# elicassion/active-gym

Hardware: NVIDIA B200
Metric: foveal_obs_per_sec (higher is better)
Workload: dtype u8

## Files before the change

active_gym_b200/csrc/agym_device.cuh:

```cuda
#pragma once
#include "agym_kernels.cuh"
#ifndef AGYM_EXPERIMENT
#define AGYM_EXPERIMENT 0
#endif

#include <cuda.h>
#include <cuda_bf16.h>
#include <cuda_fp16.h>

#include <algorithm>
#include <utility>
#include <cstdlib>
#include <cstring>

#include "../../include/agym_b200.h"

namespace agym {

namespace {


constexpr int kThreads = 256;

__device__ __forceinline__ uint4 ld_stream128(const void *p) {
// ... 126 lines not shown

__device__ __forceinline__ uint4 luma16(const uint32_t (&w)[12], uint32_t w01, uint32_t w2) {
    uint32_t acc[16];
#pragma unroll
    for (int i = 0; i < 16; ++i) {
        const int j = 3 * i, wi = j >> 2, b = j & 3;
        const uint32_t hi = wi + 1 < 12 ? w[wi + 1] : 0u;
        const uint32_t q = __byte_perm(w[wi], hi, (uint32_t)(b | (b + 1) << 4 | (b + 2) << 8 | 0x4000));
        acc[i] = __dp2a_hi(w2, q, __dp2a_lo(w01, q, 32768u));
    }
    uint32_t o[4];
#pragma unroll
    for (int m = 0; m < 4; ++m)
        o[m] = __byte_perm(__byte_perm(acc[4 * m], acc[4 * m + 1], 0x0062), __byte_perm(acc[4 * m + 2], acc[4 * m + 3], 0x0062), 0x5410);
    return make_uint4(o[0], o[1], o[2], o[3]);
}

__device__ __forceinline__ size_t align16(size_t v) { return (v + 15) & ~size_t(15); }

constexpr float kBias = 49152.5f;

__device__ void squeeze_to_cache(const DevPlan &p, const uint8_t *s_frame, float *s_t1, float *dst_global, int tid, int nt) {
    resample_w<uint8_t>(s_frame, p.S_w, s_t1, p.p_w, p.S_h, p.sq_w, tid, nt);
    __syncthreads();
    resample_h<float>(s_t1, p.p_w, dst_global, p.p_w, p.p_w, p.sq_h, tid, nt);
}

__device__ __forceinline__ uint32_t smem_u32(const void *p) { return (uint32_t)__cvta_generic_to_shared(p); }
__device__ __forceinline__ void mbar_init(uint64_t *bar, uint32_t count) {
    asm volatile("mbarrier.init.shared::cta.b64 [%0], %1;" ::"r"(smem_u32(bar)), "r"(count));
}
__device__ __forceinline__ void mbar_fence_init() { asm volatile("fence.mbarrier_init.release.cluster;" ::: "memory"); }
__device__ __forceinline__ void mbar_expect_tx(uint64_t *bar, uint32_t bytes) {
    asm volatile("mbarrier.arrive.expect_tx.shared::cta.b64 _, [%0], %1;" ::"r"(smem_u32(bar)), "r"(bytes) : "memory");
}
constexpr uint32_t kBackoffNs = 2000;
template <bool BACKOFF = false>
__device__ __forceinline__ void mbar_wait(uint64_t *bar, uint32_t parity) {
    uint32_t done = 0;
    while (!done) {
        if (BACKOFF) {
            asm volatile(
                "{\n\t.reg .pred p;\n\t"
                "mbarrier.try_wait.parity.shared::cta.b64 p, [%1], %2, %3;\n\t"
                "selp.u32 %0, 1, 0, p;\n\t}"
                : "=r"(done)
                : "r"(smem_u32(bar)), "r"(parity), "r"(kBackoffNs)
                : "memory");
        } else {
            asm volatile(
                "{\n\t.reg .pred p;\n\t"
                "mbarrier.try_wait.parity.shared::cta.b64 p, [%1], %2;\n\t"
                "selp.u32 %0, 1, 0, p;\n\t}"
                : "=r"(done)
                : "r"(smem_u32(bar)), "r"(parity)
                : "memory");
        }
    }
}
__device__ __forceinline__ void bulk_g2s(void *smem_dst, const void *gmem_src, uint32_t bytes, uint64_t *bar) {
    asm volatile("cp.async.bulk.shared::cluster.global.mbarrier::complete_tx::bytes [%0], [%1], %2, [%3];" ::"r"(
                     smem_u32(smem_dst)),
                 "l"(gmem_src), "r"(bytes), "r"(smem_u32(bar))
                 : "memory");
}

__device__ __forceinline__ void tensor_g2s_4d(void *smem_dst, const CUtensorMap *map, uint64_t *bar, int c0, int c1, int c2, int c3) {
    asm volatile("cp.async.bulk.tensor.4d.shared::cluster.global.mbarrier::complete_tx::bytes [%0], [%1, {%3, %4, %5, %6}], [%2];" ::"r"(
                     smem_u32(smem_dst)),
                 "l"(reinterpret_cast<uint64_t>(map)), "r"(smem_u32(bar)), "r"(c0), "r"(c1), "r"(c2), "r"(c3)
                 : "memory");
}

__device__ __forceinline__ void bulk_s2g(void *gmem_dst, const void *smem_src, uint32_t bytes) {
    asm volatile("cp.async.bulk.global.shared::cta.bulk_group [%0], [%1], %2;" ::"l"(gmem_dst), "r"(smem_u32(smem_src)),
                 "r"(bytes)
                 : "memory");
}
__device__ __forceinline__ void bulk_commit() { asm volatile("cp.async.bulk.commit_group;" ::: "memory"); }
template <int N>
__device__ __forceinline__ void bulk_wait_read() { asm volatile("cp.async.bulk.wait_group.read %0;" ::"n"(N) : "memory"); }
__device__ __forceinline__ void fence_async_smem() { asm volatile("fence.proxy.async.shared::cta;" ::: "memory"); }

__device__ __forceinline__ void mbar_arrive(uint64_t *bar) {
    asm volatile("mbarrier.arrive.shared::cta.b64 _, [%0];" ::"r"(smem_u32(bar)) : "memory");
}
__device__ __forceinline__ void consumer_sync() { asm volatile("bar.sync 1, %0;" ::"n"(kThreads) : "memory"); }

__device__ __forceinline__ void pdl_launch_dependents() { asm volatile("griddepcontrol.launch_dependents;" ::: "memory"); }
__device__ __forceinline__ void pdl_wait() { asm volatile("griddepcontrol.wait;" ::: "memory"); }

__device__ __forceinline__ void cp_async16(void *smem_dst, const void *gmem_src) {
    asm volatile("cp.async.cg.shared.global [%0], [%1], 16;" ::"r"((uint32_t)__cvta_generic_to_shared(smem_dst)), "l"(gmem_src));
}
__device__ __forceinline__ void cp_async16_s(uint32_t smem_addr, const void *gmem_src) {
    asm volatile("cp.async.cg.shared.global [%0], [%1], 16;" ::"r"(smem_addr), "l"(gmem_src));
}
__device__ __forceinline__ void cp_async4(void *smem_dst, const void *gmem_src) {
    asm volatile("cp.async.ca.shared.global [%0], [%1], 4;" ::"r"((uint32_t)__cvta_generic_to_shared(smem_dst)), "l"(gmem_src));
}
__device__ __forceinline__ void cp_async4_s(uint32_t smem_addr, const void *gmem_src) {
    asm volatile("cp.async.ca.shared.global [%0], [%1], 4;" ::"r"(smem_addr), "l"(gmem_src));
}
template <int SOFF, int GOFF>
__device__ __forceinline__ void cp_async4_imm(uint32_t smem_addr, const void *gmem_src) {
    asm volatile("cp.async.ca.shared.global [%0 + %2], [%1 + %3], 4;" ::"r"(smem_addr), "l"(gmem_src), "n"(SOFF), "n"(GOFF));
}
__device__ __forceinline__ void cp_async_commit() { asm volatile("cp.async.commit_group;" ::: "memory"); }
template <int N>
__device__ __forceinline__ void cp_async_wait() { asm volatile("cp.async.wait_group %0;" ::"n"(N) : "memory"); }

__device__ __forceinline__ float norm_u8(uint32_t u) {
    const float x = (float)u, r = 1.0f / 255.0f;
    const float q0 = x * r;
    return fmaf(fmaf(-q0, 255.0f, x), r, q0);
}
__device__ __forceinline__ void norm_store4(int dt, uint32_t word, void *dst, size_t index) {
    const float f0 = norm_u8(word & 0xffu), f1 = norm_u8((word >> 8) & 0xffu), f2 = norm_u8((word >> 16) & 0xffu), f3 = norm_u8(word >> 24);
    if (dt == AGYM_DTYPE_F32) {
        reinterpret_cast<float4 *>(dst)[index] = make_float4(f0, f1, f2, f3);
    } else if (dt == AGYM_DTYPE_F16) {
        const __half2 a = __floats2half2_rn(f0, f1), b = __floats2half2_rn(f2, f3);
        reinterpret_cast<uint2 *>(dst)[index] = make_uint2(*reinterpret_cast<const uint32_t *>(&a), *reinterpret_cast<const uint32_t *>(&b));
    } else {
        const __nv_bfloat162 a = __floats2bfloat162_rn(f0, f1), b = __floats2bfloat162_rn(f2, f3);
        reinterpret_cast<uint2 *>(dst)[index] = make_uint2(*reinterpret_cast<const uint32_t *>(&a), *reinterpret_cast<const uint32_t *>(&b));
    }
}
__device__ __forceinline__ void norm_store16(int dt, const uint4 v, void *dst, size_t index) {
    const uint32_t w[4] = {v.x, v.y, v.z, v.w};
    if (dt == AGYM_DTYPE_F32) {
        float4 *o = reinterpret_cast<float4 *>(dst) + 4 * index;
#pragma unroll
        for (int j = 0; j < 4; ++j)
            o[j] = make_float4(norm_u8(w[j] & 0xffu), norm_u8((w[j] >> 8) & 0xffu), norm_u8((w[j] >> 16) & 0xffu), norm_u8(w[j] >> 24));
    } else {
        uint32_t h[8];
#pragma unroll
        for (int j = 0; j < 4; ++j) {
            const float f0 = norm_u8(w[j] & 0xffu), f1 = norm_u8((w[j] >> 8) & 0xffu), f2 = norm_u8((w[j] >> 16) & 0xffu), f3 = norm_u8(w[j] >> 24);
            if (dt == AGYM_DTYPE_F16) {
                const __half2 a = __floats2half2_rn(f0, f1), b = __floats2half2_rn(f2, f3);
                h[2 * j] = *reinterpret_cast<const uint32_t *>(&a); h[2 * j + 1] = *reinterpret_cast<const uint32_t *>(&b);
            } else {
                const __nv_bfloat162 a = __floats2bfloat162_rn(f0, f1), b = __floats2bfloat162_rn(f2, f3);
                h[2 * j] = *reinterpret_cast<const uint32_t *>(&a); h[2 * j + 1] = *reinterpret_cast<const uint32_t *>(&b);
            }
        }
        uint4 *o = reinterpret_cast<uint4 *>(dst) + 2 * index;
        o[0] = make_uint4(h[0], h[1], h[2], h[3]);
        o[1] = make_uint4(h[4], h[5], h[6], h[7]);
    }
}

__device__ __forceinline__ uint64_t pack2(float lo, float hi) {
    uint64_t r;
    asm("mov.b64 %0, {%1, %2};" : "=l"(r) : "f"(lo), "f"(hi));
    return r;
}
__device__ __forceinline__ void unpack2(uint64_t v, uint32_t &lo, uint32_t &hi) {
    asm("mov.b64 {%0, %1}, %2;" : "=r"(lo), "=r"(hi) : "l"(v));
}
__device__ __forceinline__ uint64_t ffma2(uint64_t a, uint64_t b, uint64_t c) {
    uint64_t d;
    asm("fma.rn.f32x2 %0, %1, %2, %3;" : "=l"(d) : "l"(a), "l"(b), "l"(c));
    return d;
}
__device__ __forceinline__ uint64_t fsub2(uint64_t a, uint64_t b) {
    uint64_t d;
    asm("sub.rn.f32x2 %0, %1, %2;" : "=l"(d) : "l"(a), "l"(b));
// ... 43 lines not shown
```

active_gym_b200/csrc/agym_observe.cu:

```cuda
#include "agym_device.cuh"

namespace agym {

namespace {

template <int VARIANT>
__global__ void __launch_bounds__(kThreads) k_observe_fixed(const __grid_constant__ DevPlan p,
                                                            const uint8_t *__restrict__ ring,
                                                            const int32_t *__restrict__ head,
                                                            const double *__restrict__ action,
                                                            const uint8_t *__restrict__ ctrl, int32_t *__restrict__ loc,
                                                            uint8_t *__restrict__ out) {
    extern __shared__ __align__(16) uint8_t smem[];
    __shared__ int s_loc[2];
    const int n = blockIdx.x, tid = threadIdx.x;
    if (tid == 0) {
        int r, c;
        update_loc_fixed(p, n, action, ctrl, loc, r, c);
        s_loc[0] = r; s_loc[1] = c;
    }
    __syncthreads();
    const int r0 = s_loc[0], c0 = s_loc[1];
    const int h = head[n];
    const uint8_t *env_ring = ring + (size_t)n * p.K * p.plane;
// ... 473 lines not shown
            const float *s = sq + a_part * p.p_w;
            float *t = s_T + a_part * S_w + 2 * cp;
            const int sstep = parts * p.p_w, tstep = parts * S_w;
#pragma unroll 4
            for (int r = a_part; r < trows; r += parts, s += sstep, t += tstep) {
                const uint64_t u = pack2(s[a_i0], s[a_i1]), v = pack2(s[a_i0 + 1], s[a_i1 + 1]);
                *reinterpret_cast<uint64_t *>(t) = ffma2(a_w0, u, ffma2(a_w1, v, bias2));
            }
        }
        __syncthreads();

        if (active) {
            const uint32_t *fvb = reinterpret_cast<const uint32_t *>(sq + sq_words);
            const uint32_t fov_mask = word_mask(4 * q, lc, lc + p.f_w);
            const int rf = fov_mask ? lr : (1 << 29);
            const int fstride = f_h * nw_max;
            for (int k0 = 0; k0 < K; k0 += KG) {
                uint32_t *orow = out_w + ((size_t)e * K + k0) * wpp + (uint32_t)y_begin * quads + q;
                const uint32_t *fv = fvb + (k0 * f_h - rf) * nw_max + (q - (lc >> 2));
                const float *tk = s_T + (size_t)k0 * p.p_h * S_w + 4 * q;
                const int kstride = p.p_h * S_w;
                int y = y_begin, j_have = -2;
                const int2 *rp = s_row + y_begin;
                int2 rw = *rp;
                uint64_t b0[KG], b1[KG], d0[KG], d1[KG];
                while (y < y_end) {
                    const int j0 = rw.x;
#pragma unroll
                    for (int kk = 0; kk < KG; ++kk) {
                        const float *tj = tk + kk * kstride + j0 * S_w;
                        uint64_t a0, a1;
                        if (j0 == j_have + 1) { a0 = b0[kk]; a1 = b1[kk]; }
                        else { const ulonglong2 a = *reinterpret_cast<const ulonglong2 *>(tj); a0 = a.x; a1 = a.y; }
                        const ulonglong2 b = *reinterpret_cast<const ulonglong2 *>(tj + S_w);
                        b0[kk] = b.x; b1[kk] = b.y;
                        d0[kk] = fsub2(a0, b.x); d1[kk] = fsub2(a1, b.y);
                    }
                    j_have = j0;
                    do {
                        const float w0 = __int_as_float(rw.y);
                        const uint64_t w2 = pack2(w0, w0);
                        rw = *++rp;
                        uint32_t word[KG];
#pragma unroll
                        for (int kk = 0; kk < KG; ++kk) {
                            uint32_t u0, u1, u2, u3;
                            unpack2(ffma2(w2, d0[kk], b0[kk]), u0, u1);
                            unpack2(ffma2(w2, d1[kk], b1[kk]), u2, u3);
                            word[kk] = __byte_perm(__byte_perm(u0, u1, 0x0051), __byte_perm(u2, u3, 0x0051), 0x5410);
                        }
                        if ((unsigned)(y - rf) < (unsigned)f_h) {
                            const uint32_t *sh = fv + y * nw_max;
#pragma unroll
                            for (int kk = 0; kk < KG; ++kk) word[kk] = (word[kk] & ~fov_mask) | (sh[kk * fstride] & fov_mask);
                        }
#pragma unroll
                        for (int kk = 0; kk < KG; ++kk) orow[kk * wpp] = word[kk];
                        orow += quads;
                        ++y;
                    } while (rw.x == j0 && y < y_end);
                }
            }
        }
        __syncthreads();
        lr = lr1; lc = lc1; hh = hh1; hh1 = hh2;
        lr1 = s_loc[it & 1][0]; lc1 = s_loc[it & 1][1];
    }
}

struct StdGeom {
    static constexpr int S = 84, P = 20, Q = 21, SEG = 4, R = 21, SPAN = 7;
    __host__ __device__ static constexpr int src(int i) { return (40 * i - 64 + 168 * 4) / 168 - 4; }
};

template <int NW, int R0>
__device__ __forceinline__ void prefetch_rows_imm(uint32_t rows, uint32_t dst, const uint32_t *src) {
    if constexpr (R0 < StdGeom::R) {
        if (rows & (1u << R0)) cp_async4_imm<R0 * (NW ? NW : 1) * 4, R0 * StdGeom::Q * 4>(dst, src);
        prefetch_rows_imm<NW, R0 + 1>(rows, dst, src);
    }
}

template <int K, int NW, bool FS>
__global__ void __launch_bounds__(((StdGeom::Q * StdGeom::SEG * K + 31) / 32) * 32, 2)
    k_observe_peripheral_std(const __grid_constant__ DevPlan p, const __grid_constant__ ExpandStd ew,
                             const uint8_t *__restrict__ ring, const int32_t *__restrict__ head,
                             const float *__restrict__ pcache, const double *__restrict__ action,
                             const uint8_t *__restrict__ ctrl, int32_t *__restrict__ loc, uint8_t *__restrict__ out) {
    using Gm = StdGeom;
    constexpr int S = Gm::S, P = Gm::P, Q = Gm::Q, R = Gm::R;
    constexpr int NB = Q * Gm::SEG * K;
    constexpr int PP = P * P, PLANE_W = S * S / 4;
    constexpr int NBUF = 3, DIST = 2, LOC_RING = 128;
    extern __shared__ __align__(16) uint8_t smem[];
    __shared__ int4 s_loc[LOC_RING];
    __shared__ __align__(8) uint64_t full[NBUF];
    const int tid = threadIdx.x;
    const int N = p.N, f_h = p.f_h, f_w = p.f_w, G = gridDim.x;
    const int nw_max = NW ? NW : (f_w + 3) / 4 + 1;
    const int rowbuf = (f_h * Q + 9) & ~3;
    const int buf_words = K * PP + (FS ? K * rowbuf : ((K * f_h * nw_max + 3) & ~3));
    float *bufs = reinterpret_cast<float *>(smem);
    uint32_t *tiles = reinterpret_cast<uint32_t *>(bufs + NBUF * buf_words);
    const uint32_t *ring_w = reinterpret_cast<const uint32_t *>(ring);

    auto loc_batch = [&](int it0) {
        const int j = it0 + (tid & 31);
        const int env = j <= N / G + 1 ? (int)blockIdx.x + j * G : N;
        int r = 0, c = 0, hh = 0;
        if (env < N) {
            update_loc_fixed<true>(p, env, action, ctrl, loc, r, c);
            hh = head[env];
        }
        s_loc[j & (LOC_RING - 1)] = make_int4(r, c, hh, 0);
    };
    pdl_launch_dependents();
    if (tid == 0) {
        for (int i = 0; i < NBUF; ++i) mbar_init(&full[i], 1);
        mbar_fence_init();
    }

    const bool active = tid < NB;
    const int q = tid % Q, t2 = tid / Q;
    constexpr int kOrd4[16] = {7, 4, 13, 3, 0, 1, 9, 6, 10, 14, 11, 12, 8, 5, 15, 2};
    constexpr int kOrd3[12] = {11, 8, 5, 2, 9, 6, 3, 0, 10, 4, 1, 7};
    const int grp = !active ? 0 : (K == 4 ? kOrd4[t2 & 15] : (K == 3 ? kOrd3[t2 % 12] : t2));
    const int g = grp % Gm::SEG, k = grp / Gm::SEG;
    int base;
    uint64_t wa01, wa23, wb01, wb23, wc01, wc23;
    {
        const int i00 = __ldg(p.exw_i0 + 4 * q);
        base = min(i00, P - 3);
        float wa[4], wb[4], wc[4];
#pragma unroll
        for (int c = 0; c < 4; ++c) {
            const int sel = __ldg(p.exw_i0 + 4 * q + c) - base;
            const float w0 = __ldg(p.exw_w0 + 4 * q + c), w1 = __ldg(p.exw_w1 + 4 * q + c);
            wa[c] = sel == 0 ? w0 : 0.f;
            wb[c] = sel == 0 ? w1 : w0;
            wc[c] = sel == 0 ? 0.f : w1;
        }
        wa01 = pack2(wa[0], wa[1]); wa23 = pack2(wa[2], wa[3]);
        wb01 = pack2(wb[0], wb[1]); wb23 = pack2(wb[2], wb[3]);
        wc01 = pack2(wc[0], wc[1]); wc23 = pack2(wc[2], wc[3]);
    }
    const uint64_t bias2 = pack2(kBias, kBias);
    const int row_first = 5 * g - 1;
    const int so_t0 = (row_first < 0 ? 0 : row_first) * P + base;
    const int so_mid = row_first * P + base;
    const int so_t6 = (row_first + 6 > P - 1 ? P - 1 : row_first + 6) * P + base;
    const uint32_t bufs_s = smem_u32(bufs);
    const uint32_t word0 = (uint32_t)(g * R) * Q + q;
    constexpr int NJ = 2;
    int ck_row[NJ], ck_k[NJ], ck_c4[NJ];
    if constexpr (FS) {
        const int cpr = (f_w + 14) / 16 + 1, total = K * f_h * cpr;
#pragma unroll
        for (int a = 0; a < NJ; ++a) {
            const int i = tid + a * (int)blockDim.x;
            const int row = i / cpr, kk = row / f_h;
            ck_k[a] = i < total ? kk : -1;
            ck_row[a] = (row - kk * f_h) * Q;
            ck_c4[a] = (i - row * cpr) * 4;
        }
    }

    auto fovea_rows = [&](int lr, int lc, uint32_t &mask) {
        mask = word_mask(4 * q, lc, lc + f_w);
        const int r_lo = lr - g * R;
        const int m_lo = max(r_lo, 0), m_hi = min(r_lo + f_h, R);
        return (mask && m_hi > m_lo) ? (((1u << m_hi) - 1u) & ~((1u << m_lo) - 1u)) : 0u;
    };
    auto fovea_pos = [&](int lr, int lc) { return (k * f_h + g * R - lr) * nw_max + (q - (lc >> 2)); };
    auto prefetch = [&](int env, int j) {
        const int b = j % NBUF;
        if (tid == 0) {
            mbar_expect_tx(&full[b], K * PP * 4);
            bulk_g2s(bufs + b * buf_words, pcache + (size_t)env * (K * PP), K * PP * 4, &full[b]);
        }
        if constexpr (FS) {
            const int4 lh = s_loc[j & (LOC_RING - 1)];
            const int top = lh.x * Q, wb = top & ~3;
            const int lw = lh.y >> 2, lastw = (lh.y + f_w - 1) >> 2;
#pragma unroll
            for (int a = 0; a < NJ; ++a) {
                if (ck_k[a] < 0) continue;
                const int rowbase = top + ck_row[a];
                const int cw = ((rowbase + lw) & ~3) + ck_c4[a];
                if (cw > rowbase + lastw) continue;
                int slot = lh.z + 1 + ck_k[a];
                slot -= slot >= K ? K : 0;
                cp_async16_s(bufs_s + (uint32_t)(b * buf_words + K * PP + ck_k[a] * rowbuf + (cw - wb)) * 4u,
                             ring_w + ((size_t)env * K + slot) * PLANE_W + cw);
            }
        } else if (active) {
            const int4 lh = s_loc[j & (LOC_RING - 1)];
            uint32_t mask;
            const uint32_t rows = fovea_rows(lh.x, lh.y, mask);
            if (rows) {
                int slot = lh.z + 1 + k;
                slot -= slot >= K ? K : 0;
                const uint32_t *src = ring_w + ((size_t)env * K + slot) * PLANE_W + word0;
                const uint32_t dst = bufs_s + (uint32_t)(b * buf_words + K * PP + fovea_pos(lh.x, lh.y)) * 4u;
                if (NW) {
                    prefetch_rows_imm<NW, 0>(rows, dst, src);
                } else {
#pragma unroll
                    for (int r = 0; r < R; ++r)
                        if (rows & (1u << r)) cp_async4_s(dst + (uint32_t)(r * nw_max) * 4u, src + r * Q);
                }
            }
        }
    };
    auto t_row = [&](const float *sq, int so, uint64_t &t01, uint64_t &t23) {
        const float s0 = sq[so], s1 = sq[so + 1], s2 = sq[so + 2];
        const uint64_t p0 = pack2(s0, s0), p1 = pack2(s1, s1), p2 = pack2(s2, s2);
        t01 = ffma2(p2, wc01, ffma2(p1, wb01, ffma2(p0, wa01, bias2)));
        t23 = ffma2(p2, wc23, ffma2(p1, wb23, ffma2(p0, wa23, bias2)));
    };

    pdl_wait();
    if (tid < 32) loc_batch(0);
    __syncthreads();
    {
        const int e0 = blockIdx.x;
#pragma unroll
        for (int j = 0; j < DIST; ++j) {
            if (e0 + j * G < N) prefetch(e0 + j * G, j);
            cp_async_commit();
        }
        if constexpr (FS) {
            cp_async_wait<DIST - 1>();
            __syncthreads();
        }
    }
    int it = 0;
    for (int e = blockIdx.x; e < N; e += G, ++it) {
        if (e + DIST * G < N) prefetch(e + DIST * G, it + DIST);
        cp_async_commit();
        if ((it & 31) == 0 && tid < 32) loc_batch(it + 32);
        const int b = it % NBUF;
        if constexpr (!FS) cp_async_wait<DIST>();
        mbar_wait(&full[b], (it / NBUF) & 1);
        uint32_t *tile = tiles + (it & 1) * (K * PLANE_W);
        if (active) {
            const int4 lh = s_loc[it & (LOC_RING - 1)];
            uint32_t fov_mask;
            const uint32_t rows = fovea_rows(lh.x, lh.y, fov_mask);
            int slot = lh.z + 1 + k;
            slot -= slot >= K ? K : 0;
            const float *sq = bufs + b * buf_words + slot * PP;
            const uint32_t *sh = reinterpret_cast<const uint32_t *>(bufs + b * buf_words + K * PP) +
                                 (FS ? k * rowbuf + (int)word0 - ((lh.x * Q) & ~3) : fovea_pos(lh.x, lh.y));
            constexpr int SHP = FS ? Q : 0;
            uint32_t *o = tile + k * PLANE_W + word0;
            uint64_t a0, a1, b0, b1, d0 = 0, d1 = 0;
            t_row(sq, so_t0, a0, a1);
            t_row(sq, so_mid + P, b0, b1);
            int t_have = 0;
#pragma unroll
            for (int r = 0; r < R; ++r) {
                const int t = Gm::src(r) + 1;
                if (t != t_have) {
                    a0 = b0; a1 = b1;
                    t_row(sq, t + 1 == Gm::SPAN - 1 ? so_t6 : so_mid + (t + 1) * P, b0, b1);
                    t_have = t;
                }
                if (r == 0 || Gm::src(r) != Gm::src(r - 1)) { d0 = fsub2(a0, b0); d1 = fsub2(a1, b1); }
                const uint64_t w2 = pack2(ew.hw[r], ew.hw[r]);
                uint32_t u0, u1, u2, u3;
                unpack2(ffma2(w2, d0, b0), u0, u1);
                unpack2(ffma2(w2, d1, b1), u2, u3);
                uint32_t word = __byte_perm(__byte_perm(u0, u1, 0x0051), __byte_perm(u2, u3, 0x0051), 0x5410);
                if (rows & (1u << r))
                    word = (word & ~fov_mask) | (sh[FS ? r * SHP : r * nw_max] & fov_mask);
                o[r * Q] = word;
            }
        }
        fence_async_smem();
        if (tid == 0) bulk_wait_read<0>();
        if constexpr (FS) cp_async_wait<DIST - 1>();
        __syncthreads();
        if (tid == 0) {
            bulk_s2g(out + (size_t)e * (K * PLANE_W * 4), tile, K * PLANE_W * 4);
            bulk_commit();
        }
        if (p.norm_out) {
            const uint4 *t4 = reinterpret_cast<const uint4 *>(tile);
            for (int i = tid; i < K * PLANE_W / 4; i += (int)blockDim.x)
                norm_store16(p.norm_dt, t4[i], p.norm_out, (size_t)e * (K * PLANE_W / 4) + i);
        }
    }
    if (tid == 0) bulk_wait_read<0>();
}


}

namespace {
cudaError_t normalize_after(cudaError_t e, const uint8_t *out, size_t bytes, void *norm_out, int norm_dt, cudaStream_t st) {
    if (e != cudaSuccess || !norm_out) return e;
    if (bytes % 16 != 0) return cudaErrorInvalidValue;
    return launch_normalize(out, bytes, norm_dt, norm_out, st);
}
}

cudaError_t launch_observe_fixed(const DevPlan &p0, const uint8_t *ring, const int32_t *head, const double *action,
                                 const uint8_t *ctrl, int32_t *loc, int variant, uint8_t *out, void *norm_out, int norm_dt,
                                 cudaStream_t st) {
    DevPlan p = p0;
    p.norm_out = norm_out; p.norm_dt = norm_dt;
    const size_t out_bytes = (size_t)p.N * p.K * (variant == AGYM_OUT_CROP ? p.f_h * p.f_w : p.plane);
    cudaError_t e;
    const int crop_nwx = (p.f_w + 2) / 4 + 1;
    const size_t crop_smem = a16((size_t)(p.K * p.f_h * p.f_w / 4) * 8) + (size_t)kCropWarps * p.K * p.f_h * crop_nwx * 4;
    CropV3Args c3;
    c3.nch = (p.f_w + 30) / 16;
    c3.g = p.f_w % 4 == 0 ? 1 : p.f_w % 2 == 0 ? 2 : 4;
    c3.gw = c3.g * p.f_w / 4;
    c3.ngroups = p.K * p.f_h / c3.g;
    c3.m_fh = 0xFFFFFFFFu / (uint32_t)p.f_h + 1u;
    c3.slice = (int)(16 + (size_t)p.K * p.f_h * c3.nch * 16);
    const int c3_warps = (p.C == 3 && (size_t)kCrop3Warps * (c3.slice + (size_t)p.K * p.f_h * p.f_w) > 100 * 1024) ? 4 : kCrop3Warps;
    const size_t crop3_smem = (size_t)c3_warps * (c3.slice + (size_t)p.K * p.f_h * p.f_w);
    if (variant == AGYM_OUT_CROP && (p.K * p.f_h * p.f_w) % 4 == 0 && (p.K * p.f_h) % c3.g == 0 && p.plane % 16 == 0 &&
        (reinterpret_cast<uintptr_t>(ring) & 15) == 0 && (reinterpret_cast<uintptr_t>(out) & 3) == 0 &&
        !g_disable_std && !g_crop_old && !g_crop_v2 && crop3_smem <= 100 * 1024) {
        const int grid = (p.N + c3_warps - 1) / c3_warps;
#define AGYM_LAUNCH_CROP3(FW, W)                                                                                  \
    {                                                                                                             \
        if ((e = set_smem(k_observe_fixed_crop_v3<FW, W>, crop3_smem)) != cudaSuccess) return e;                   \
        k_observe_fixed_crop_v3<FW, W><<<grid, W * 32, crop3_smem, st>>>(p, ring, head, action, ctrl, loc, out, c3); \
    }
        if (c3_warps == 4) {
            if (p.f_w == 30) AGYM_LAUNCH_CROP3(30, 4)
            else AGYM_LAUNCH_CROP3(0, 4)
        } else if (p.f_w == 30) AGYM_LAUNCH_CROP3(30, kCrop3Warps)
        else AGYM_LAUNCH_CROP3(0, kCrop3Warps)
#undef AGYM_LAUNCH_CROP3
        return cudaGetLastError();
    }
    if (variant == AGYM_OUT_CROP && (p.K * p.f_h * p.f_w) % 4 == 0 && !g_disable_std && !g_crop_old &&
        crop_smem <= 64 * 1024 && p.K * p.f_h * crop_nwx * 4 + 4 < 65536) {
        if ((e = set_smem(k_observe_fixed_crop_v2, crop_smem)) != cudaSuccess) return e;
        k_observe_fixed_crop_v2<<<(p.N + kCropWarps - 1) / kCropWarps, kCropWarps * 32, crop_smem, st>>>(p, ring, head, action, ctrl, loc, out, crop_nwx);
        return cudaGetLastError();
    } else if (variant == AGYM_OUT_CROP && (p.K * p.f_h * p.f_w) % 4 == 0 && !g_disable_std) {
        k_observe_fixed_crop_warp<<<(p.N + kThreads / 32 - 1) / (kThreads / 32), kThreads, 0, st>>>(p, ring, head, action, ctrl, loc, out);
    } else if (variant == AGYM_OUT_CROP) {
        k_observe_fixed<AGYM_OUT_CROP><<<p.N, kThreads, 0, st>>>(p, ring, head, action, ctrl, loc, out);
    } else if (variant == AGYM_OUT_MASK) {
        k_observe_fixed<AGYM_OUT_MASK><<<p.N, kThreads, 0, st>>>(p, ring, head, action, ctrl, loc, out);
    } else {
        const size_t smem = sizeof(float) * ((size_t)p.f_h * p.f_w + (size_t)p.f_h * p.S_w);
        if ((e = set_smem(k_observe_fixed<AGYM_OUT_RESIZE_FULL>, smem)) != cudaSuccess) return e;
        k_observe_fixed<AGYM_OUT_RESIZE_FULL><<<p.N, kThreads, smem, st>>>(p, ring, head, action, ctrl, loc, out);
    }
    return normalize_after(cudaGetLastError(), out, out_bytes, norm_out, norm_dt, st);
}

cudaError_t launch_observe_peripheral(const DevPlan &p0, const ExpandStd *ew, const uint8_t *ring, const int32_t *head,
                                      const float *pcache, const double *action, const uint8_t *ctrl, int32_t *loc,
                                      uint8_t *out, void *norm_out, int norm_dt, cudaStream_t st) {
    DevPlan p = p0;
    p.norm_out = norm_out; p.norm_dt = norm_dt;
    const size_t out_bytes = (size_t)p.N * p.K * p.plane;
    const size_t smem = a16(p.plane) + sizeof(float) * ((size_t)p.S_h * p.p_w + (size_t)p.p_h * p.p_w + (size_t)p.p_h * p.S_w);
    cudaError_t e;
    const int quads = p.S_w / 4;
    if (pcache && ew && ew->ok && (p.K == 4 || p.K == 3) && !g_disable_std && p.N < (1 << 30) &&
        (reinterpret_cast<uintptr_t>(out) & 15) == 0 && (reinterpret_cast<uintptr_t>(pcache) & 15) == 0) {
        const int nw_max = (p.f_w + 3) / 4 + 1;
        const size_t fov_words = ((size_t)p.K * p.f_h * nw_max + 3) & ~size_t(3);
        size_t fs = 4 * (3 * ((size_t)p.K * 400 + fov_words) + 2 * (size_t)p.K * 1764);
        const size_t fs_rows = 4 * (3 * ((size_t)p.K * 400 + (size_t)p.K * ((p.f_h * 21 + 9) & ~3)) + 2 * (size_t)p.K * 1764);
        const int std_threads = ((21 * 4 * p.K + 31) / 32) * 32;
        const bool full_rows = !g_std_nofs && fs_rows <= 112 * 1024 && p.K * p.f_h * ((p.f_w + 14) / 16 + 1) <= 2 * std_threads;
        int dev = 0, sms = 148, occ = 0;
        cudaGetDevice(&dev);
        cudaDeviceGetAttribute(&sms, cudaDevAttrMultiProcessorCount, dev);
#define AGYM_LAUNCH_STD(KK, NW, FSV)                                                                               \
    {                                                                                                              \
    if (fs <= 220 * 1024) {                                                                                        \
        const int threads = ((21 * 4 * KK + 31) / 32) * 32;                                                        \
        if ((e = set_smem(k_observe_peripheral_std<KK, NW, FSV>, fs)) != cudaSuccess) return e;                    \
        cudaOccupancyMaxActiveBlocksPerMultiprocessor(&occ, k_observe_peripheral_std<KK, NW, FSV>, threads, fs);   \
        if (occ >= 1) {                                                                                            \
            return launch_pdl(k_observe_peripheral_std<KK, NW, FSV>, dim3(std::min(p.N, sms * occ)), dim3(threads), fs, st, \
                              p, *ew, ring, head, pcache, action, ctrl, loc, out);                                 \
        }                                                                                                          \
    }                                                                                                              \
    }
        if (full_rows) {
            fs = fs_rows;
            if (p.K == 4) AGYM_LAUNCH_STD(4, 0, true)
            else AGYM_LAUNCH_STD(3, 0, true)
        }
        else if (p.K == 4 && nw_max == 9) AGYM_LAUNCH_STD(4, 9, false)
        else if (p.K == 4) AGYM_LAUNCH_STD(4, 0, false)
        else if (nw_max == 9) AGYM_LAUNCH_STD(3, 9, false)
        else AGYM_LAUNCH_STD(3, 0, false)
#undef AGYM_LAUNCH_STD
    }
    if (pcache && p.fast_expand && quads <= 64 && (p.p_h * p.p_w) % 4 == 0) {
        int ysegs = std::max(1, 128 / quads);
        {
            int g = p.S_h, b2 = p.p_h;
            while (b2) { const int t = g % b2; g = b2; b2 = t; }
            const int period = p.S_h / g;
            while (ysegs > 1 && (p.S_h % ysegs != 0 || (p.S_h / ysegs) % period != 0)) --ysegs;
        }
        const int threads = ((std::max(quads * ysegs, 2 * quads) + 31) / 32) * 32;
        const int nw_max = (p.f_w + 3) / 4 + 1;
        const size_t buf_words = (((size_t)p.K * p.p_h * p.p_w + 3) & ~size_t(3)) + (((size_t)p.K * p.f_h * nw_max + 3) & ~size_t(3));
        const size_t fs = 4 * (2 * buf_words + (size_t)p.K * p.p_h * p.S_w) + 8 * ((size_t)p.S_h + 1);
        int dev = 0, sms = 148, occ = 1;
        cudaGetDevice(&dev);
        cudaDeviceGetAttribute(&sms, cudaDevAttrMultiProcessorCount, dev);
#define AGYM_LAUNCH_PF(KG, PW)                                                                                     \
    {                                                                                                              \
        if ((e = set_smem(k_observe_peripheral_v2<KG, PW>, fs)) != cudaSuccess) return e;                          \
        cudaOccupancyMaxActiveBlocksPerMultiprocessor(&occ, k_observe_peripheral_v2<KG, PW>, threads, fs);         \
        if (occ < 1) return cudaErrorInvalidConfiguration;                                                         \
        k_observe_peripheral_v2<KG, PW><<<std::min(p.N, sms * occ), threads, fs, st>>>(p, ring, head, pcache, action, \
                                                                                      ctrl, loc, out, ysegs);     \
    }
        if (p.K == 4 && p.plane == 7056) AGYM_LAUNCH_PF(4, 1764)
        else if (p.K == 3 && p.plane == 7056) AGYM_LAUNCH_PF(3, 1764)
        else if (p.C == 3 && p.K % 3 == 0 && p.plane == 7056) AGYM_LAUNCH_PF(3, 1764)
        else if (p.K % 4 == 0) AGYM_LAUNCH_PF(4, 0)
        else if (p.K % 3 == 0) AGYM_LAUNCH_PF(3, 0)
        else if (p.K % 2 == 0) AGYM_LAUNCH_PF(2, 0)
        else AGYM_LAUNCH_PF(1, 0)
#undef AGYM_LAUNCH_PF
        return normalize_after(cudaGetLastError(), out, out_bytes, norm_out, norm_dt, st);
    }
    if (pcache) {
        if ((e = set_smem(k_observe_peripheral<true>, smem)) != cudaSuccess) return e;
        k_observe_peripheral<true><<<p.N, kThreads, smem, st>>>(p, ring, head, pcache, action, ctrl, loc, out);
    } else {
        if ((e = set_smem(k_observe_peripheral<false>, smem)) != cudaSuccess) return e;
        k_observe_peripheral<false><<<p.N, kThreads, smem, st>>>(p, ring, head, pcache, action, ctrl, loc, out);
    }
    return normalize_after(cudaGetLastError(), out, out_bytes, norm_out, norm_dt, st);
}


}
```

Baseline: 51.58 million.

## Warp-specialize peripheral observe kernel with a producer warp and mbarrier pipeline

Adds a dedicated producer warp to the peripheral std kernel. It issues the bulk squeeze loads and the bulk tile stores, and it waits on per-tile done/free mbarriers, so the consumers no longer block on a CTA-wide __syncthreads per environment. Fovea cp.async staging now signals the full barrier through cp.async.mbarrier.arrive.noinc instead of commit/wait groups. Normalized output is fused into the expand loop as per-word stores rather than a second pass over the tile. This adds an extra warp per block and more barrier bookkeeping, and it risks lower occupancy or subtle phase and ordering bugs.

```diff
diff --git a/active_gym_b200/csrc/agym_device.cuh b/active_gym_b200/csrc/agym_device.cuh
--- a/active_gym_b200/csrc/agym_device.cuh
+++ b/active_gym_b200/csrc/agym_device.cuh
@@ -232,6 +232,9 @@
 __device__ __forceinline__ void bulk_wait_read() { asm volatile("cp.async.bulk.wait_group.read %0;" ::"n"(N) : "memory"); }
 __device__ __forceinline__ void fence_async_smem() { asm volatile("fence.proxy.async.shared::cta;" ::: "memory"); }
 
+__device__ __forceinline__ void cp_async_mbar_arrive_noinc(uint64_t *bar) {
+    asm volatile("cp.async.mbarrier.arrive.noinc.shared::cta.b64 [%0];" ::"r"(smem_u32(bar)) : "memory");
+}
 __device__ __forceinline__ void mbar_arrive(uint64_t *bar) {
     asm volatile("mbarrier.arrive.shared::cta.b64 _, [%0];" ::"r"(smem_u32(bar)) : "memory");
 }
diff --git a/active_gym_b200/csrc/agym_observe.cu b/active_gym_b200/csrc/agym_observe.cu
--- a/active_gym_b200/csrc/agym_observe.cu
+++ b/active_gym_b200/csrc/agym_observe.cu
@@ -579,7 +579,7 @@
 }
 
 template <int K, int NW, bool FS>
-__global__ void __launch_bounds__(((StdGeom::Q * StdGeom::SEG * K + 31) / 32) * 32, 2)
+__global__ void __launch_bounds__(((StdGeom::Q * StdGeom::SEG * K + 31) / 32) * 32 + 32, 2)
     k_observe_peripheral_std(const __grid_constant__ DevPlan p, const __grid_constant__ ExpandStd ew,
                              const uint8_t *__restrict__ ring, const int32_t *__restrict__ head,
                              const float *__restrict__ pcache, const double *__restrict__ action,
@@ -587,11 +587,12 @@
     using Gm = StdGeom;
     constexpr int S = Gm::S, P = Gm::P, Q = Gm::Q, R = Gm::R;
     constexpr int NB = Q * Gm::SEG * K;
+    constexpr int NCT = ((NB + 31) / 32) * 32;
     constexpr int PP = P * P, PLANE_W = S * S / 4;
-    constexpr int NBUF = 3, DIST = 2, LOC_RING = 128;
+    constexpr int NBUF = 3, LOC_RING = 128;
     extern __shared__ __align__(16) uint8_t smem[];
     __shared__ int4 s_loc[LOC_RING];
-    __shared__ __align__(8) uint64_t full[NBUF];
+    __shared__ __align__(8) uint64_t full[NBUF], done[2], tfree[2];
     const int tid = threadIdx.x;
     const int N = p.N, f_h = p.f_h, f_w = p.f_w, G = gridDim.x;
     const int nw_max = NW ? NW : (f_w + 3) / 4 + 1;
@@ -613,8 +614,39 @@
     };
     pdl_launch_dependents();
     if (tid == 0) {
-        for (int i = 0; i < NBUF; ++i) mbar_init(&full[i], 1);
+        for (int i = 0; i < NBUF; ++i) mbar_init(&full[i], NCT + 1);
+        for (int i = 0; i < 2; ++i) { mbar_init(&done[i], NCT / 32); mbar_init(&tfree[i], 1); }
         mbar_fence_init();
+    }
+    auto squeeze_g2s = [&](int env, int j) {
+        const int b = j % NBUF;
+        mbar_expect_tx(&full[b], K * PP * 4);
+        bulk_g2s(bufs + b * buf_words, pcache + (size_t)env * (K * PP), K * PP * 4, &full[b]);
+    };
+
+    if (tid >= NCT) {
+        const bool lead = tid == NCT;
+        pdl_wait();
+        loc_batch(0);
+        __syncthreads();
+        if (lead)
+            for (int j = 0; j < NBUF; ++j)
+                if ((int)blockIdx.x + j * G < N) squeeze_g2s(blockIdx.x + j * G, j);
+        int j = 0;
+        for (int e = blockIdx.x; e < N; e += G, ++j) {
+            if ((j & 31) == 0) loc_batch(j + 32);
+            if (lead) {
+                const int t = j & 1;
+                mbar_wait<true>(&done[t], (j >> 1) & 1);
+                bulk_s2g(out + (size_t)e * (K * PLANE_W * 4), tiles + t * (K * PLANE_W), K * PLANE_W * 4);
+                bulk_commit();
+                if (e + NBUF * G < N) squeeze_g2s(e + NBUF * G, j + NBUF);
+                bulk_wait_read<0>();
+                mbar_arrive(&tfree[t]);
+            }
+            __syncwarp();
+        }
+        return;
     }
 
     const bool active = tid < NB;
@@ -654,7 +686,7 @@
         const int cpr = (f_w + 14) / 16 + 1, total = K * f_h * cpr;
 #pragma unroll
         for (int a = 0; a < NJ; ++a) {
-            const int i = tid + a * (int)blockDim.x;
+            const int i = tid + a * NCT;
             const int row = i / cpr, kk = row / f_h;
             ck_k[a] = i < total ? kk : -1;
             ck_row[a] = (row - kk * f_h) * Q;
@@ -669,12 +701,8 @@
         return (mask && m_hi > m_lo) ? (((1u << m_hi) - 1u) & ~((1u << m_lo) - 1u)) : 0u;
     };
     auto fovea_pos = [&](int lr, int lc) { return (k * f_h + g * R - lr) * nw_max + (q - (lc >> 2)); };
-    auto prefetch = [&](int env, int j) {
+    auto stage_fovea = [&](int env, int j) {
         const int b = j % NBUF;
-        if (tid == 0) {
-            mbar_expect_tx(&full[b], K * PP * 4);
-            bulk_g2s(bufs + b * buf_words, pcache + (size_t)env * (K * PP), K * PP * 4, &full[b]);
-        }
         if constexpr (FS) {
             const int4 lh = s_loc[j & (LOC_RING - 1)];
             const int top = lh.x * Q, wb = top & ~3;
@@ -708,6 +736,7 @@
                 }
             }
         }
+        cp_async_mbar_arrive_noinc(&full[b]);
     };
     auto t_row = [&](const float *sq, int so, uint64_t &t01, uint64_t &t23) {
         const float s0 = sq[so], s1 = sq[so + 1], s2 = sq[so + 2];
@@ -715,80 +744,70 @@
         t01 = ffma2(p2, wc01, ffma2(p1, wb01, ffma2(p0, wa01, bias2)));
         t23 = ffma2(p2, wc23, ffma2(p1, wb23, ffma2(p0, wa23, bias2)));
     };
+    auto expand = [&](auto norm_c, int e, int it, const float *buf, uint32_t *tile) {
+        constexpr bool NORM = decltype(norm_c)::value;
+        const int4 lh = s_loc[it & (LOC_RING - 1)];
+        uint32_t fov_mask;
+        const uint32_t rows = fovea_rows(lh.x, lh.y, fov_mask);
+        int slot = lh.z + 1 + k;
+        slot -= slot >= K ? K : 0;
+        const float *sq = buf + slot * PP;
+        const uint32_t *sh = reinterpret_cast<const uint32_t *>(buf + K * PP) +
+                             (FS ? k * rowbuf + (int)word0 - ((lh.x * Q) & ~3) : fovea_pos(lh.x, lh.y));
+        constexpr int SHP = FS ? Q : 0;
+        uint32_t *o = tile + k * PLANE_W + word0;
+        const size_t nidx = ((size_t)e * K + k) * PLANE_W + word0;
+        uint64_t a0, a1, b0, b1, d0 = 0, d1 = 0;
+        t_row(sq, so_t0, a0, a1);
+        t_row(sq, so_mid + P, b0, b1);
+        int t_have = 0;
+#pragma unroll
+        for (int r = 0; r < R; ++r) {
+            const int t = Gm::src(r) + 1;
+            if (t != t_have) {
+                a0 = b0; a1 = b1;
+                t_row(sq, t + 1 == Gm::SPAN - 1 ? so_t6 : so_mid + (t + 1) * P, b0, b1);
+                t_have = t;
+            }
+            if (r == 0 || Gm::src(r) != Gm::src(r - 1)) { d0 = fsub2(a0, b0); d1 = fsub2(a1, b1); }
+            const uint64_t w2 = pack2(ew.hw[r], ew.hw[r]);
+            uint32_t u0, u1, u2, u3;
+            unpack2(ffma2(w2, d0, b0), u0, u1);
+            unpack2(ffma2(w2, d1, b1), u2, u3);
+            uint32_t word = __byte_perm(__byte_perm(u0, u1, 0x0051), __byte_perm(u2, u3, 0x0051), 0x5410);
+            if (rows & (1u << r))
+                word = (word & ~fov_mask) | (sh[FS ? r * SHP : r * nw_max] & fov_mask);
+            o[r * Q] = word;
+            if constexpr (NORM) norm_store4(p.norm_dt, word, p.norm_out, nidx + r * Q);
+        }
+    };
 
     pdl_wait();
-    if (tid < 32) loc_batch(0);
     __syncthreads();
     {
         const int e0 = blockIdx.x;
-#pragma unroll
-        for (int j = 0; j < DIST; ++j) {
-            if (e0 + j * G < N) prefetch(e0 + j * G, j);
-            cp_async_commit();
-        }
-        if constexpr (FS) {
-            cp_async_wait<DIST - 1>();
-            __syncthreads();
-        }
-    }
+        for (int j = 0; j < 2; ++j)
+            if (e0 + j * G < N) stage_fovea(e0 + j * G, j);
+    }
+    const int lane = tid & 31;
     int it = 0;
     for (int e = blockIdx.x; e < N; e += G, ++it) {
-        if (e + DIST * G < N) prefetch(e + DIST * G, it + DIST);
-        cp_async_commit();
-        if ((it & 31) == 0 && tid < 32) loc_batch(it + 32);
+        if (e + 2 * G < N) {
+            if (it >= 1) mbar_wait(&done[(it - 1) & 1], ((it - 1) >> 1) & 1);
+            stage_fovea(e + 2 * G, it + 2);
+        }
+        const int t = it & 1;
+        if (it >= 2) mbar_wait(&tfree[t], ((it >> 1) - 1) & 1);
         const int b = it % NBUF;
-        if constexpr (!FS) cp_async_wait<DIST>();
         mbar_wait(&full[b], (it / NBUF) & 1);
-        uint32_t *tile = tiles + (it & 1) * (K * PLANE_W);
         if (active) {
-            const int4 lh = s_loc[it & (LOC_RING - 1)];
-            uint32_t fov_mask;
-            const uint32_t rows = fovea_rows(lh.x, lh.y, fov_mask);
-            int slot = lh.z + 1 + k;
-            slot -= slot >= K ? K : 0;
-            const float *sq = bufs + b * buf_words + slot * PP;
-            const uint32_t *sh = reinterpret_cast<const uint32_t *>(bufs + b * buf_words + K * PP) +
-                                 (FS ? k * rowbuf + (int)word0 - ((lh.x * Q) & ~3) : fovea_pos(lh.x, lh.y));
-            constexpr int SHP = FS ? Q : 0;
-            uint32_t *o = tile + k * PLANE_W + word0;
-            uint64_t a0, a1, b0, b1, d0 = 0, d1 = 0;
-            t_row(sq, so_t0, a0, a1);
-            t_row(sq, so_mid + P, b0, b1);
-            int t_have = 0;
-#pragma unroll
-            for (int r = 0; r < R; ++r) {
-                const int t = Gm::src(r) + 1;
-                if (t != t_have) {
-                    a0 = b0; a1 = b1;
-                    t_row(sq, t + 1 == Gm::SPAN - 1 ? so_t6 : so_mid + (t + 1) * P, b0, b1);
-                    t_have = t;
-                }
-                if (r == 0 || Gm::src(r) != Gm::src(r - 1)) { d0 = fsub2(a0, b0); d1 = fsub2(a1, b1); }
-                const uint64_t w2 = pack2(ew.hw[r], ew.hw[r]);
-                uint32_t u0, u1, u2, u3;
-                unpack2(ffma2(w2, d0, b0), u0, u1);
-                unpack2(ffma2(w2, d1, b1), u2, u3);
-                uint32_t word = __byte_perm(__byte_perm(u0, u1, 0x0051), __byte_perm(u2, u3, 0x0051), 0x5410);
-                if (rows & (1u << r))
-                    word = (word & ~fov_mask) | (sh[FS ? r * SHP : r * nw_max] & fov_mask);
-                o[r * Q] = word;
-            }
+            if (p.norm_out) expand(std::true_type{}, e, it, bufs + b * buf_words, tiles + t * (K * PLANE_W));
+            else expand(std::false_type{}, e, it, bufs + b * buf_words, tiles + t * (K * PLANE_W));
         }
         fence_async_smem();
-        if (tid == 0) bulk_wait_read<0>();
-        if constexpr (FS) cp_async_wait<DIST - 1>();
-        __syncthreads();
-        if (tid == 0) {
-            bulk_s2g(out + (size_t)e * (K * PLANE_W * 4), tile, K * PLANE_W * 4);
-            bulk_commit();
-        }
-        if (p.norm_out) {
-            const uint4 *t4 = reinterpret_cast<const uint4 *>(tile);
-            for (int i = tid; i < K * PLANE_W / 4; i += (int)blockDim.x)
-                norm_store16(p.norm_dt, t4[i], p.norm_out, (size_t)e * (K * PLANE_W / 4) + i);
-        }
-    }
-    if (tid == 0) bulk_wait_read<0>();
+        __syncwarp();
+        if (lane == 0) mbar_arrive(&done[t]);
+    }
 }
 
 
@@ -879,7 +898,7 @@
 #define AGYM_LAUNCH_STD(KK, NW, FSV)                                                                               \
     {                                                                                                              \
     if (fs <= 220 * 1024) {                                                                                        \
-        const int threads = ((21 * 4 * KK + 31) / 32) * 32;                                                        \
+        const int threads = ((21 * 4 * KK + 31) / 32) * 32 + 32;                                                        \
         if ((e = set_smem(k_observe_peripheral_std<KK, NW, FSV>, fs)) != cudaSuccess) return e;                    \
         cudaOccupancyMaxActiveBlocksPerMultiprocessor(&occ, k_observe_peripheral_std<KK, NW, FSV>, threads, fs);   \
         if (occ >= 1) {                                                                                            \
```

Result: faster. 52.76 million (median of 6 runs) (+2.3%).

## Split peripheral kernel into independent per-frame warp groups with named barriers

Applied to the files above, without the earlier changes.

Restructures the standard peripheral observe kernel so each of the K stacked frames is handled by its own 96-thread group, with per-group shared buffers, per-group mbarriers, per-frame bulk loads and per-frame bulk stores. Block-wide __syncthreads in the main loop are replaced by named barriers per group, and the shared location ring is coordinated through full/free mbarriers. The aim is to let frame groups progress independently and avoid whole-block stalls, at the cost of more threads per block (some idle lanes), smaller bulk transfers, and more complex barrier bookkeeping.

```diff
diff --git a/active_gym_b200/csrc/agym_device.cuh b/active_gym_b200/csrc/agym_device.cuh
--- a/active_gym_b200/csrc/agym_device.cuh
+++ b/active_gym_b200/csrc/agym_device.cuh
@@ -236,6 +236,8 @@
     asm volatile("mbarrier.arrive.shared::cta.b64 _, [%0];" ::"r"(smem_u32(bar)) : "memory");
 }
 __device__ __forceinline__ void consumer_sync() { asm volatile("bar.sync 1, %0;" ::"n"(kThreads) : "memory"); }
+template <int THREADS>
+__device__ __forceinline__ void named_sync(int id) { asm volatile("bar.sync %0, %1;" ::"r"(id), "n"(THREADS) : "memory"); }
 
 __device__ __forceinline__ void pdl_launch_dependents() { asm volatile("griddepcontrol.launch_dependents;" ::: "memory"); }
 __device__ __forceinline__ void pdl_wait() { asm volatile("griddepcontrol.wait;" ::: "memory"); }
diff --git a/active_gym_b200/csrc/agym_observe.cu b/active_gym_b200/csrc/agym_observe.cu
--- a/active_gym_b200/csrc/agym_observe.cu
+++ b/active_gym_b200/csrc/agym_observe.cu
@@ -579,29 +579,34 @@
 }
 
 template <int K, int NW, bool FS>
-__global__ void __launch_bounds__(((StdGeom::Q * StdGeom::SEG * K + 31) / 32) * 32, 2)
+__global__ void __launch_bounds__(96 * K, 2)
     k_observe_peripheral_std(const __grid_constant__ DevPlan p, const __grid_constant__ ExpandStd ew,
                              const uint8_t *__restrict__ ring, const int32_t *__restrict__ head,
                              const float *__restrict__ pcache, const double *__restrict__ action,
                              const uint8_t *__restrict__ ctrl, int32_t *__restrict__ loc, uint8_t *__restrict__ out) {
     using Gm = StdGeom;
     constexpr int S = Gm::S, P = Gm::P, Q = Gm::Q, R = Gm::R;
-    constexpr int NB = Q * Gm::SEG * K;
+    constexpr int GT = 96;
     constexpr int PP = P * P, PLANE_W = S * S / 4;
-    constexpr int NBUF = 3, DIST = 2, LOC_RING = 128;
+    constexpr int NBUF = 3, DIST = 2, LOC_RING = 128, LOC_BATCHES = LOC_RING / 32;
     extern __shared__ __align__(16) uint8_t smem[];
     __shared__ int4 s_loc[LOC_RING];
-    __shared__ __align__(8) uint64_t full[NBUF];
+    __shared__ __align__(8) uint64_t full[K][NBUF];
+    __shared__ __align__(8) uint64_t loc_full[LOC_BATCHES], loc_free[LOC_BATCHES];
     const int tid = threadIdx.x;
+    const int k = tid / GT, lt = tid - k * GT;
+    const bool lead = lt == 0;
     const int N = p.N, f_h = p.f_h, f_w = p.f_w, G = gridDim.x;
     const int nw_max = NW ? NW : (f_w + 3) / 4 + 1;
     const int rowbuf = (f_h * Q + 9) & ~3;
-    const int buf_words = K * PP + (FS ? K * rowbuf : ((K * f_h * nw_max + 3) & ~3));
-    float *bufs = reinterpret_cast<float *>(smem);
+    const int buf_words = PP + (FS ? rowbuf : ((f_h * nw_max + 3) & ~3));
+    float *bufs = reinterpret_cast<float *>(smem) + k * (NBUF * buf_words + 2 * PLANE_W);
     uint32_t *tiles = reinterpret_cast<uint32_t *>(bufs + NBUF * buf_words);
     const uint32_t *ring_w = reinterpret_cast<const uint32_t *>(ring);
 
     auto loc_batch = [&](int it0) {
+        const int bt = it0 / 32;
+        if (bt >= LOC_BATCHES) mbar_wait(&loc_free[bt % LOC_BATCHES], (bt / LOC_BATCHES - 1) & 1);
         const int j = it0 + (tid & 31);
         const int env = j <= N / G + 1 ? (int)blockIdx.x + j * G : N;
         int r = 0, c = 0, hh = 0;
@@ -610,19 +615,20 @@
             hh = head[env];
         }
         s_loc[j & (LOC_RING - 1)] = make_int4(r, c, hh, 0);
+        mbar_arrive(&loc_full[bt % LOC_BATCHES]);
     };
     pdl_launch_dependents();
     if (tid == 0) {
-        for (int i = 0; i < NBUF; ++i) mbar_init(&full[i], 1);
+        for (int i = 0; i < K * NBUF; ++i) mbar_init(&full[i / NBUF][i % NBUF], 1);
+        for (int i = 0; i < LOC_BATCHES; ++i) {
+            mbar_init(&loc_full[i], 32);
+            mbar_init(&loc_free[i], K);
+        }
         mbar_fence_init();
     }
 
-    const bool active = tid < NB;
-    const int q = tid % Q, t2 = tid / Q;
-    constexpr int kOrd4[16] = {7, 4, 13, 3, 0, 1, 9, 6, 10, 14, 11, 12, 8, 5, 15, 2};
-    constexpr int kOrd3[12] = {11, 8, 5, 2, 9, 6, 3, 0, 10, 4, 1, 7};
-    const int grp = !active ? 0 : (K == 4 ? kOrd4[t2 & 15] : (K == 3 ? kOrd3[t2 % 12] : t2));
-    const int g = grp % Gm::SEG, k = grp / Gm::SEG;
+    const bool active = lt < Q * Gm::SEG;
+    const int q = lt % Q, g = (lt / Q + 3) & 3;
     int base;
     uint64_t wa01, wa23, wb01, wb23, wc01, wc23;
     {
@@ -649,15 +655,13 @@
     const uint32_t bufs_s = smem_u32(bufs);
     const uint32_t word0 = (uint32_t)(g * R) * Q + q;
     constexpr int NJ = 2;
-    int ck_row[NJ], ck_k[NJ], ck_c4[NJ];
+    int ck_row[NJ], ck_c4[NJ];
     if constexpr (FS) {
-        const int cpr = (f_w + 14) / 16 + 1, total = K * f_h * cpr;
+        const int cpr = (f_w + 14) / 16 + 1, total = f_h * cpr;
 #pragma unroll
         for (int a = 0; a < NJ; ++a) {
-            const int i = tid + a * (int)blockDim.x;
-            const int row = i / cpr, kk = row / f_h;
-            ck_k[a] = i < total ? kk : -1;
-            ck_row[a] = (row - kk * f_h) * Q;
+            const int i = lt + a * GT, row = i / cpr;
+            ck_row[a] = i < total ? row * Q : -1;
             ck_c4[a] = (i - row * cpr) * 4;
         }
     }
@@ -668,37 +672,35 @@
         const int m_lo = max(r_lo, 0), m_hi = min(r_lo + f_h, R);
         return (mask && m_hi > m_lo) ? (((1u << m_hi) - 1u) & ~((1u << m_lo) - 1u)) : 0u;
     };
-    auto fovea_pos = [&](int lr, int lc) { return (k * f_h + g * R - lr) * nw_max + (q - (lc >> 2)); };
+    auto fovea_pos = [&](int lr, int lc) { return (g * R - lr) * nw_max + (q - (lc >> 2)); };
     auto prefetch = [&](int env, int j) {
         const int b = j % NBUF;
-        if (tid == 0) {
-            mbar_expect_tx(&full[b], K * PP * 4);
-            bulk_g2s(bufs + b * buf_words, pcache + (size_t)env * (K * PP), K * PP * 4, &full[b]);
-        }
+        if ((j & 31) == 0) mbar_wait(&loc_full[(j / 32) % LOC_BATCHES], (j / 32 / LOC_BATCHES) & 1);
+        const int4 lh = s_loc[j & (LOC_RING - 1)];
+        int slot = lh.z + 1 + k;
+        slot -= slot >= K ? K : 0;
+        if (lead) {
+            mbar_expect_tx(&full[k][b], PP * 4);
+            bulk_g2s(bufs + b * buf_words, pcache + ((size_t)env * K + slot) * PP, PP * 4, &full[k][b]);
+        }
+        const uint32_t *plane = ring_w + ((size_t)env * K + slot) * PLANE_W;
         if constexpr (FS) {
-            const int4 lh = s_loc[j & (LOC_RING - 1)];
             const int top = lh.x * Q, wb = top & ~3;
             const int lw = lh.y >> 2, lastw = (lh.y + f_w - 1) >> 2;
 #pragma unroll
             for (int a = 0; a < NJ; ++a) {
-                if (ck_k[a] < 0) continue;
+                if (ck_row[a] < 0) continue;
                 const int rowbase = top + ck_row[a];
                 const int cw = ((rowbase + lw) & ~3) + ck_c4[a];
                 if (cw > rowbase + lastw) continue;
-                int slot = lh.z + 1 + ck_k[a];
-                slot -= slot >= K ? K : 0;
-                cp_async16_s(bufs_s + (uint32_t)(b * buf_words + K * PP + ck_k[a] * rowbuf + (cw - wb)) * 4u,
-                             ring_w + ((size_t)env * K + slot) * PLANE_W + cw);
+                cp_async16_s(bufs_s + (uint32_t)(b * buf_words + PP + (cw - wb)) * 4u, plane + cw);
             }
         } else if (active) {
-            const int4 lh = s_loc[j & (LOC_RING - 1)];
             uint32_t mask;
             const uint32_t rows = fovea_rows(lh.x, lh.y, mask);
             if (rows) {
-                int slot = lh.z + 1 + k;
-                slot -= slot >= K ? K : 0;
-                const uint32_t *src = ring_w + ((size_t)env * K + slot) * PLANE_W + word0;
-                const uint32_t dst = bufs_s + (uint32_t)(b * buf_words + K * PP + fovea_pos(lh.x, lh.y)) * 4u;
+                const uint32_t *src = plane + word0;
+                const uint32_t dst = bufs_s + (uint32_t)(b * buf_words + PP + fovea_pos(lh.x, lh.y)) * 4u;
                 if (NW) {
                     prefetch_rows_imm<NW, 0>(rows, dst, src);
                 } else {
@@ -717,8 +719,8 @@
     };
 
     pdl_wait();
+    __syncthreads();
     if (tid < 32) loc_batch(0);
-    __syncthreads();
     {
         const int e0 = blockIdx.x;
 #pragma unroll
@@ -728,7 +730,7 @@
         }
         if constexpr (FS) {
             cp_async_wait<DIST - 1>();
-            __syncthreads();
+            named_sync<GT>(1 + k);
         }
     }
     int it = 0;
@@ -738,19 +740,17 @@
         if ((it & 31) == 0 && tid < 32) loc_batch(it + 32);
         const int b = it % NBUF;
         if constexpr (!FS) cp_async_wait<DIST>();
-        mbar_wait(&full[b], (it / NBUF) & 1);
-        uint32_t *tile = tiles + (it & 1) * (K * PLANE_W);
+        mbar_wait(&full[k][b], (it / NBUF) & 1);
+        uint32_t *tile = tiles + (it & 1) * PLANE_W;
         if (active) {
             const int4 lh = s_loc[it & (LOC_RING - 1)];
             uint32_t fov_mask;
             const uint32_t rows = fovea_rows(lh.x, lh.y, fov_mask);
-            int slot = lh.z + 1 + k;
-            slot -= slot >= K ? K : 0;
-            const float *sq = bufs + b * buf_words + slot * PP;
-            const uint32_t *sh = reinterpret_cast<const uint32_t *>(bufs + b * buf_words + K * PP) +
-                                 (FS ? k * rowbuf + (int)word0 - ((lh.x * Q) & ~3) : fovea_pos(lh.x, lh.y));
+            const float *sq = bufs + b * buf_words;
+            const uint32_t *sh = reinterpret_cast<const uint32_t *>(bufs + b * buf_words + PP) +
+                                 (FS ? (int)word0 - ((lh.x * Q) & ~3) : fovea_pos(lh.x, lh.y));
             constexpr int SHP = FS ? Q : 0;
-            uint32_t *o = tile + k * PLANE_W + word0;
+            uint32_t *o = tile + word0;
             uint64_t a0, a1, b0, b1, d0 = 0, d1 = 0;
             t_row(sq, so_t0, a0, a1);
             t_row(sq, so_mid + P, b0, b1);
@@ -775,20 +775,21 @@
             }
         }
         fence_async_smem();
-        if (tid == 0) bulk_wait_read<0>();
+        if (lead) bulk_wait_read<0>();
         if constexpr (FS) cp_async_wait<DIST - 1>();
-        __syncthreads();
-        if (tid == 0) {
-            bulk_s2g(out + (size_t)e * (K * PLANE_W * 4), tile, K * PLANE_W * 4);
+        named_sync<GT>(1 + k);
+        if (lead) {
+            if ((it & 31) == 31) mbar_arrive(&loc_free[(it / 32) % LOC_BATCHES]);
+            bulk_s2g(out + ((size_t)e * K + k) * (PLANE_W * 4), tile, PLANE_W * 4);
             bulk_commit();
         }
         if (p.norm_out) {
             const uint4 *t4 = reinterpret_cast<const uint4 *>(tile);
-            for (int i = tid; i < K * PLANE_W / 4; i += (int)blockDim.x)
-                norm_store16(p.norm_dt, t4[i], p.norm_out, (size_t)e * (K * PLANE_W / 4) + i);
-        }
-    }
-    if (tid == 0) bulk_wait_read<0>();
+            for (int i = lt; i < PLANE_W / 4; i += GT)
+                norm_store16(p.norm_dt, t4[i], p.norm_out, ((size_t)e * K + k) * (PLANE_W / 4) + i);
+        }
+    }
+    if (lead) bulk_wait_read<0>();
 }
 
 
@@ -868,9 +869,9 @@
     if (pcache && ew && ew->ok && (p.K == 4 || p.K == 3) && !g_disable_std && p.N < (1 << 30) &&
         (reinterpret_cast<uintptr_t>(out) & 15) == 0 && (reinterpret_cast<uintptr_t>(pcache) & 15) == 0) {
         const int nw_max = (p.f_w + 3) / 4 + 1;
-        const size_t fov_words = ((size_t)p.K * p.f_h * nw_max + 3) & ~size_t(3);
-        size_t fs = 4 * (3 * ((size_t)p.K * 400 + fov_words) + 2 * (size_t)p.K * 1764);
-        const size_t fs_rows = 4 * (3 * ((size_t)p.K * 400 + (size_t)p.K * ((p.f_h * 21 + 9) & ~3)) + 2 * (size_t)p.K * 1764);
+        const size_t fov_words = ((size_t)p.f_h * nw_max + 3) & ~size_t(3);
+        size_t fs = 4 * (size_t)p.K * (3 * (400 + fov_words) + 2 * 1764);
+        const size_t fs_rows = 4 * (size_t)p.K * (3 * (400 + (size_t)((p.f_h * 21 + 9) & ~3)) + 2 * 1764);
         const int std_threads = ((21 * 4 * p.K + 31) / 32) * 32;
         const bool full_rows = !g_std_nofs && fs_rows <= 112 * 1024 && p.K * p.f_h * ((p.f_w + 14) / 16 + 1) <= 2 * std_threads;
         int dev = 0, sms = 148, occ = 0;
@@ -879,7 +880,7 @@
 #define AGYM_LAUNCH_STD(KK, NW, FSV)                                                                               \
     {                                                                                                              \
     if (fs <= 220 * 1024) {                                                                                        \
-        const int threads = ((21 * 4 * KK + 31) / 32) * 32;                                                        \
+        const int threads = 96 * KK;                                               \
         if ((e = set_smem(k_observe_peripheral_std<KK, NW, FSV>, fs)) != cudaSuccess) return e;                    \
         cudaOccupancyMaxActiveBlocksPerMultiprocessor(&occ, k_observe_peripheral_std<KK, NW, FSV>, threads, fs);   \
         if (occ >= 1) {                                                                                            \
```

Result: faster. 51.62 million before, 53.32 million after (median of 6 runs) (+3.3%).
